# SmallVCM/SmallVCM

Hardware: AMD Instinct MI355X
Metric: Mpaths/sec (light+camera), VCM scene 1 at 2048^2 (higher is better)
Workload: dtype f32; 1 GPU; scene 1 -a vcm 2048x2048 maxPathLength 10 minPathLength 0 radiusFactor 0.003 radiusAlpha 0.75 seed 1234, iterations 5..408 timed; parallelism=1 renderer(s) (iteration-parallel, smallvcm.cxx:61-108) on one GPU, 1 in flight

## Files before the change

### smallvcm_amd/csrc/vcm_api.hip

```cpp
#include <hip/hip_runtime.h>
#include <stdio.h>
#include <stdlib.h>
#include <string.h>
#include <string>
#include <new>
#include <mutex>
#include <vector>
#include <condition_variable>
#include <atomic>

#include "vcm_kernels.h"
#include "vcm_kat.h"
#include "scene_host.h"
#include "vcm_denoise.h"
#include "vcm_variance.h"

using namespace vcm;

static thread_local std::string g_err;
static thread_local bool g_hipFailed;
static int fail(const char *what, const char *detail)
{
    g_err = std::string(what) + ": " + (detail ? detail : "");
    return -1;
// ... 188 lines not shown

static thread_local size_t g_allocBytes;
template <typename T> static int dalloc(T **p, size_t n)
{
    void *v = NULL;
    HIPCHK(hipMalloc(&v, (n ? n : 1) * sizeof(T)));
    g_allocBytes += (n ? n : 1) * sizeof(T);
    *p = (T *)v;
    return 0;
}
#define DFREE(p) do { if (p) { (void)hipFree(p); p = NULL; } } while (0)

static std::mutex g_arenaRegistryMutex;
static ArenaPool *g_pools[64];

static Arena *arena_new(int device, ArenaPool *pool)
{
    Arena *a = new Arena();
    a->device = device;
    memset((void *)&a->s, 0, sizeof(Scratch));
    a->capLocal = a->capN = 0; a->capS = a->capL = 0; a->capSharded = false; a->bytes = 0;
    a->allocated = false; a->eventReady = a->lastValid = false; a->lastUser = NULL;
    a->pool = pool; a->ownerThread = 0; a->busy = false;
    a->mtx = pool ? &pool->m : &a->ownMtx;
    a->cv = pool ? &pool->cv : &a->ownCv;
    return a;
}
static ArenaPool *pool_get(int device)
{
    if (device < 0 || device >= 64) return NULL;
    std::lock_guard<std::mutex> g(g_arenaRegistryMutex);
    if (!g_pools[device]) {
        ArenaPool *p = new ArenaPool();
        p->device = device; p->users = 0; p->count = 0;
        memset(p->arenas, 0, sizeof(p->arenas));
        const char *e = getenv("SMALLVCM_AMD_ARENAS");
        p->limit = (e && atoi(e) > 0) ? (atoi(e) < VCM_MAX_ARENAS ? atoi(e) : VCM_MAX_ARENAS) : 0;
        g_pools[device] = p;
    }
    return g_pools[device];
}

static void arena_free_buffers(Arena *a)
{
    Scratch &s = a->s;
    DFREE(s.store.v); DFREE(s.store.count); DFREE(s.store.lenMask);
    DFREE(s.dPathStart); DFREE(s.dLocalTotal); DFREE(s.dTileSums[0]); DFREE(s.dTileSums[1]); DFREE(s.dTileSums[2]); DFREE(s.dTileSums[3]);
    DFREE(s.dPixCount); DFREE(s.dPixStart); DFREE(s.dSplatArrival); DFREE(s.dSplatList);
    DFREE(s.dRecordsLocal); DFREE(s.dRecordsAll); DFREE(s.dSlotOfVertex); DFREE(s.dSplat);
    DFREE(s.dCellCount); DFREE(s.dCellStart); DFREE(s.dCellId); DFREE(s.dUnsorted); DFREE(s.dRadixHist);
    DFREE(s.dGx); DFREE(s.dGy); DFREE(s.dGz); DFREE(s.dGb); DFREE(s.dG1); DFREE(s.dG2); DFREE(s.dG3); DFREE(s.dSortedIndex);
    DFREE(s.dCamOut); DFREE(s.dCamMask);
    DFREE(s.vs.q); DFREE(s.vs.q4); DFREE(s.vs.meta); DFREE(s.vs.count);
    DFREE(s.vs.diTask); DFREE(s.vs.vcTask); DFREE(s.vs.diOut); DFREE(s.vs.vcOut); DFREE(s.vs.mergeOut);
    DFREE(s.dQueryKey); DFREE(s.dSortedVertex); DFREE(s.dQueryStart); DFREE(s.dQueryCount); DFREE(s.dQueryArrival);
    a->allocated = false;
    a->capLocal = a->capN = 0; a->capS = a->capL = 0; a->capSharded = false;
}

static int arena_ensure(Arena *a, size_t nLocal, size_t N, int S, int L, bool sharded)
{
    if (!a->eventReady) { HIPCHK(hipEventCreateWithFlags(&a->lastUse, hipEventDisableTiming)); a->eventReady = true; }
    if (a->allocated && nLocal <= a->capLocal && N <= a->capN && S <= a->capS && L <= a->capL && (!sharded || a->capSharded))
        return 0;
    HIPCHK(hipDeviceSynchronize());
    const size_t cl = nLocal > a->capLocal ? nLocal : a->capLocal, cn = N > a->capN ? N : a->capN;
    const int cs = S > a->capS ? S : a->capS, cL = L > a->capL ? L : a->capL;
    const bool sh = sharded || a->capSharded;
    arena_free_buffers(a);
    a->lastValid = false;
    a->lastUser = NULL;
    a->bytes = 0;
    const size_t bytesBefore = g_allocBytes;
    Scratch &s = a->s;
    const size_t slots = (size_t)cs * cl;
    const size_t allRecs = (size_t)cs * cn;
    if (dalloc(&s.store.v, slots * VCM_LV_FIELDS) || dalloc(&s.store.count, cl) || dalloc(&s.store.lenMask, cl)) return -1;
    if (dalloc(&s.dPathStart, cl + 1) || dalloc(&s.dLocalTotal, 1)) return -1;
    size_t maxScan = (cn > cl ? cn : cl) + 1;
    if (maxScan < (size_t)VCM_QSORT_BUCKETS + 1) maxScan = (size_t)VCM_QSORT_BUCKETS + 1;
    for (int w = 0; w < 4; w++) if (dalloc(&s.dTileSums[w], maxScan / VCM_SCAN_TILE + 2)) return -1;
    if (dalloc(&s.dRecordsLocal, slots * VCM_MERGE_RECORD_FLOATS)) return -1;
    if (dalloc(&s.dSlotOfVertex, slots) || dalloc(&s.dSplat, slots)) return -1;
    if (dalloc(&s.dPixCount, cn + 2) || dalloc(&s.dPixStart, cn + 2) || dalloc(&s.dSplatArrival, slots) || dalloc(&s.dSplatList, slots)) return -1;
    if (sh && dalloc(&s.dRecordsAll, allRecs * VCM_MERGE_RECORD_FLOATS)) return -1;
    if (dalloc(&s.dCellCount, cn + 2) || dalloc(&s.dCellStart, cn + 2)) return -1;
    if (dalloc(&s.dCellId, allRecs) || dalloc(&s.dUnsorted, allRecs) || dalloc(&s.dRadixHist, (size_t)2 * 256 * VCM_RSORT_MAX_BLOCKS)) return -1;
    if (dalloc(&s.dGx, allRecs + VCM_MERGE_UNROLL) || dalloc(&s.dGy, allRecs + VCM_MERGE_UNROLL) ||
        dalloc(&s.dGz, allRecs + VCM_MERGE_UNROLL) || dalloc(&s.dGb, 3 * (allRecs + 2 * VCM_MERGE_UNROLL)) || dalloc(&s.dG1, allRecs) || dalloc(&s.dG2, allRecs) ||
        dalloc(&s.dG3, allRecs) || dalloc(&s.dSortedIndex, allRecs)) return -1;
    if (dalloc(&s.dCamOut, cl) || dalloc(&s.dCamMask, cl) || dalloc(&s.vs.count, 32)) return -1;
    const size_t maxWaves = (size_t)VCM_MAX_TRACE_WAVES;
    const size_t vitems = (size_t)(cL > 0 ? cL : 1) * cl;
    const size_t vslots = vitems + vitems / 3 + maxWaves * VCM_QBLOCK_VERTEX;
    const size_t vcPerPath = (cL >= 3) ? (size_t)(cL - 1) * (size_t)(cL - 2) / 2 : 1;
    const size_t vcslots = 2 * vcPerPath * cl + maxWaves * VCM_QBLOCK_VC;
    s.vs.qcap = vslots;
    if (dalloc(&s.vs.q, vslots * 4) || dalloc(&s.vs.q4, vslots) || dalloc(&s.vs.meta, vslots) ||
        dalloc(&s.vs.diTask, vslots) || dalloc(&s.vs.diOut, vslots) ||
        dalloc(&s.vs.mergeOut, vslots) || dalloc(&s.vs.vcTask, 2 * vcslots) || dalloc(&s.vs.vcOut, vcslots) ||
        dalloc(&s.dQueryKey, vslots) || dalloc(&s.dSortedVertex, vslots)) return -1;
    const size_t qsN = (cn > (size_t)VCM_QSORT_BUCKETS ? cn : (size_t)VCM_QSORT_BUCKETS) + 2;
    if (dalloc(&s.dQueryStart, qsN) || dalloc(&s.dQueryCount, (size_t)VCM_QSORT_BUCKETS + 2) ||
        dalloc(&s.dQueryArrival, vslots)) return -1;
    a->capLocal = cl; a->capN = cn; a->capS = cs; a->capL = cL; a->capSharded = sh;
    a->allocated = true;
    a->bytes = g_allocBytes - bytesBefore;
    return 0;
}

static bool pool_may_grow(ArenaPool *p)
{
    if (p->count >= VCM_MAX_ARENAS) return false;
    if (p->limit > 0) return p->count < p->limit;
    if (p->count == 0) return true;
    size_t held = 0, largest = 0;
    for (int i = 0; i < p->count; i++) { held += p->arenas[i]->bytes; if (p->arenas[i]->bytes > largest) largest = p->arenas[i]->bytes; }
    size_t freeB = 0, totalB = 0;
    if (hipMemGetInfo(&freeB, &totalB) != hipSuccess) return false;
    return held + largest <= totalB / 4 && largest + (totalB / 16) <= freeB;
}

static int arena_acquire(vcm_ctx *c, int S, int L)
{
    Arena *a = NULL;
    bool wait;
    if (c->pool) {
        ArenaPool *p = c->pool;
        std::unique_lock<std::mutex> lk(p->m);
        for (;;) {
            Arena *mine = NULL, *idle = NULL, *lru = NULL;
            bool holdsOne = false;
            for (int i = 0; i < p->count; i++) {
                Arena *x = p->arenas[i];
                if (x->busy) { if (x->ownerThread == this_thread_id()) holdsOne = true; continue; }
                if (x->lastUser == c) mine = x;
                else if (!x->lastValid || hipEventQuery(x->lastUse) == hipSuccess) idle = x;
                else lru = x;
            }
            (void)hipGetLastError();
            a = mine ? mine : idle;
            if (!a && pool_may_grow(p)) { a = arena_new(p->device, p); p->arenas[p->count++] = a; }
            if (!a) a = lru;
            if (a) break;
            if (holdsOne)
                return fail("vcm_begin_iteration", "this thread is already inside an iteration on this device and no further "
                                                   "scratch arena is free: single-rank contexts share the iteration scratch, "
                                                   "end an iteration first (or raise vcm_set_arena_limit)");
            p->cv.wait(lk);
        }
        a->busy = true;
        a->ownerThread = this_thread_id();
        wait = a->lastValid && a->lastUser != c;
// ... 1098 lines not shown
        if (!c->P.wavefront && join_grid(c)) return -1;
    } else {
        if (mark(c, EV_GRID_K0)) return -1;
        if (mark(c, EV_GRID)) return -1;
    }
    return 0;
}

static GridStore grid_of(vcm_ctx *c)
{
    GridStore grid;
    grid.cellStart = c->dCellStart; grid.gx = c->dGx; grid.gy = c->dGy; grid.gz = c->dGz; grid.gb = c->dGb; grid.g1 = c->dG1; grid.g2 = c->dG2; grid.g3 = c->dG3;
    grid.hdr = c->dHdr;
    return grid;
}

static int vcm_trace_camera_impl(vcm_ctx *c)
{
    if (!c || !c->inIteration) return fail("vcm_trace_camera", "no iteration in progress");
    if (use_device(c)) return -1;
    if (flush_light_splats(c)) return -1;
    c->cameraTraced = true;
    if (c->lightTraceOnly) return 0;
    int blocks, chunk;
    trace_launch_shape(c->nLocal, &blocks, &chunk);
    if (c->resolveInFlight) HIPCHK(hipStreamWaitEvent(c->stream, c->evResolved, 0));
    if (mark(c, EV_CAMERA_K0)) return -1;
    if (c->renderer) {
        if (c->renderer == 1)
            LAUNCH_SC_CAM_PICK(c, k_path_trace, dim3(blocks), dim3(VCM_TRACE_BLOCK), 0, c->stream, c->dScene, c->P, c->dCamOut,
                               c->dRngCam, c->dStats, chunk, take_stamps(c, c->stream), c->vs.count + 8);
        else
            LAUNCH_SC_CAM(c, k_eye_light, dim3(2048), dim3(256), 0, c->stream, c->dScene, c->P, c->dCamOut, c->dRngCam,
                               c->dStats, take_stamps(c, c->stream));
        HIPCHK(hipGetLastError());
        if (mark(c, EV_CAMERA_K1)) return -1;
        if (mark(c, EV_CONNECT_K1)) return -1;
        return 0;
    }
    if (c->P.wavefront) {
        c->countedInCamera = c->useVM && (c->gridBuilt || c->bboxPreset);
        c->vs.sortHdr = c->countedInCamera ? c->dHdr : NULL;
        c->vs.sortKey = c->countedInCamera ? c->dQueryKey : NULL;
        c->vs.sortArrival = c->countedInCamera ? c->dQueryArrival : NULL;
        c->vs.bucketCount = c->countedInCamera ? c->dQueryCount : NULL;
        if (c->countedInCamera) {
            if (c->prezeroed) HIPCHK(hipStreamWaitEvent(c->stream, c->evZero, 0));
            else if (zero_ranges(c->stream, c->dQueryCount, ((size_t)c->P.nBuckets + 1) * sizeof(int))) return -1;
        }
        LAUNCH_SC_MODE_CAM_PICK(c, k_camera_trace, 1, dim3(blocks), dim3(VCM_TRACE_BLOCK), 0, c->stream, c->dScene, c->P,
                           c->store, grid_of(c), c->vs, c->dCamOut, c->dCamMask, c->dRngCam, c->dStats, chunk, take_stamps(c, c->stream));
        if (mark(c, EV_CAMERA_K1)) return -1;
        if (c->useVC) {
            c->scatteredInDI = c->countedInCamera && c->P.minLen <= 2;
            const bool inlineSort = c->scatteredInDI && (c->nLocal <= (1 << 20) || grid_sort_is_radix(c));
            if (c->countedInCamera && c->world == 1 && !inlineSort) {
                HIPCHK(hipEventRecord(c->evSortFork, c->stream));
                HIPCHK(hipStreamWaitEvent(c->side, c->evSortFork, 0));
                const StampArgs none = { { NULL, NULL, NULL, NULL } };
                if (launch_scan_on<int>(c, 3, c->side, c->dQueryCount, c->P.nBuckets, c->dQueryStart, NULL, 1, none)) return -1;
                hipLaunchKernelGGL(k_query_scatter, dim3(aux_blocks(c->nLocal)), dim3(256), 0, c->side, c->vs, (const int *)c->dQueryKey,
                                   (const int *)c->dQueryArrival, (const int *)c->dQueryStart, c->dSortedVertex);
                HIPCHK(hipEventRecord(c->evSorted, c->side));
                c->sortInFlight = true;
                c->scatteredInDI = false;
            }
            if (c->scatteredInDI && launch_scan<int>(c, c->dQueryCount, c->P.nBuckets, c->dQueryStart, NULL, 1)) return -1;
            {
                HIPCHK(hipEventRecord(c->evSplatFork, c->stream));
                HIPCHK(hipStreamWaitEvent(c->splat, c->evSplatFork, 0));
                LAUNCH_SC(c, k_connect_vc, dim3(task_blocks(c->nLocal)), dim3(VCM_TASK_BLOCK), 0, c->splat, c->dScene, c->P, c->vs,
                                   c->store, c->dStats);
                HIPCHK(hipEventRecord(c->evSplatDone, c->splat));
                c->splatInFlight = true;
            }
            LAUNCH_SC_PICK(c, k_connect_di, dim3(task_blocks(c->nLocal)), dim3(VCM_TASK_BLOCK), 0, c->stream, c->dScene, c->P, c->vs,
                               c->dStats, c->scatteredInDI ? (const int *)c->dQueryStart : (const int *)NULL,
                               c->scatteredInDI ? c->dSortedVertex : (int *)NULL, take_stamps(c, c->stream));
        }
        if (mark(c, EV_CONNECT_K1)) return -1;
    } else {
        if (c->useVM && !c->gridBuilt) return fail("vcm_trace_camera", "strict mode merges inside the camera pass: call vcm_build_grid first");
        LAUNCH_SC_MODE_CAM_PICK(c, k_camera_trace, 0, dim3(blocks), dim3(VCM_TRACE_BLOCK), 0, c->stream, c->dScene, c->P,
                           c->store, grid_of(c), c->vs, c->dCamOut, c->dCamMask, c->dRngCam, c->dStats, chunk, take_stamps(c, c->stream));
        if (mark(c, EV_CAMERA_K1)) return -1;
        if (mark(c, EV_CONNECT_K1)) return -1;
    }
    HIPCHK(hipGetLastError());
    if (c->world > 1 && flush_stamps(c, c->stream)) return -1;
    return 0;
}

#define VCM_SPACE_BLOCKS 512
static int space_scratch(vcm_ctx *c)
{
    if (c->dSpaceMatrix) return 0;
    HIPCHK(hipMalloc((void **)&c->dSpaceMatrix, sizeof(int) * VCM_SPACE_MAX_SLABS * VCM_SPACE_BLOCKS));
    HIPCHK(hipMalloc((void **)&c->dSpaceScanned, sizeof(int) * (VCM_SPACE_MAX_SLABS * VCM_SPACE_BLOCKS + 1)));
    HIPCHK(hipMalloc((void **)&c->dSpaceTotals, sizeof(int) * VCM_SPACE_MAX_SLABS));
    HIPCHK(hipMalloc((void **)&c->dSpaceHist, sizeof(int) * 256));
    return 0;
}
static int space_ready(vcm_ctx *c, const char *who)
{
    if (!c || !c->inIteration) return fail(who, "no iteration in progress");
    if (c->world <= 1) return fail(who, "the context is not sharded");
    if (!c->useVM || !c->P.wavefront) return fail(who, "needs a merging algorithm in wavefront mode");
// ... 1032 lines not shown
```

### smallvcm_amd/csrc/vcm_core.h

```cpp
#ifndef SMALLVCM_AMD_VCM_CORE_H
#define SMALLVCM_AMD_VCM_CORE_H

#include "../../include/smallvcm_amd.h"
#include "vcm_math.h"
#include "detmath.h"
#include "philox.h"

namespace vcm {

struct IterParams {
    uint32_t seed, localIter;
    uint32_t minLen, maxLen;
    int   resX, resY, N;
    int   p0, nLocal;
    int   S;
    int   useVM, useVC, lightTraceOnly, ppm;
    float radius, radiusSqr, vmNormalization, misVmWeightFactor, misVcWeightFactor;
    float lightSubPathCount;
    float cellSize, invCellSize;
    int   nCells;
    int   wavefront;
    int   renderer;
    int   iteration;
    int   qblockVertex, qblockDI, qblockVC;
    int   nBuckets;
    int   foreignOut;
};

struct GridHeader {
    uint32_t bboxMinU[3], bboxMaxU[3];
    float bboxMin[3], bboxMax[3];
    int   nRecords;
    int   nLocalRecords;
    int   pad[2];
};

#define VCM_LV_FIELDS 4
struct LightStore {
    F4 *v;
    unsigned char *count;
    uint32_t *lenMask;
};
VCM_HD F4 &lv(const LightStore &s, size_t slot, int k) { return s.v[slot * VCM_LV_FIELDS + (size_t)k]; }

struct alignas(8) F2 { float x, y; };
struct GridStore {
    const int *cellStart;
    const float *gx, *gy, *gz;
    const float *gb;
    const F4 *g1;
    const F4 *g2;
    const F2 *g3;
    const GridHeader *hdr;
};

VCM_HD size_t grid_blocked_index(int i, int axis) { return (size_t)(i >> 2) * 12u + (size_t)(axis * 4 + (i & 3)); }

struct alignas(16) I4 { int x, y, z, w; };
struct VertexStore {
    F4 *q, *q4;
    size_t qcap;
    I4 *meta;
    int *count;
    int *diTask;
    int *vcTask;
    F4 *diOut;
    F4 *vcOut;
    F4 *mergeOut;
    const GridHeader *sortHdr;
    int *sortKey, *sortArrival, *bucketCount;
};
struct alignas(8) VcTaskPair { int vertex, j; };
VCM_HD F4 &vq(const VertexStore &vs, int k, size_t i) { return k < 4 ? vs.q[i * 4 + (size_t)k] : vs.q4[i]; }
VCM_HD size_t path_slot(const IterParams &P, uint32_t pathLength, uint32_t lp)
{
    return (size_t)(pathLength - 1u) * (size_t)P.nLocal + (size_t)lp;
}
VCM_HD size_t merge_out_slot(const IterParams &P, uint32_t pathLength, uint32_t lp, int vi)
{
    return P.foreignOut ? (size_t)vi : path_slot(P, pathLength, lp);
}

struct LaneStats {
    uint32_t lightRays, cameraRays, shadowRays, mergeQueries, mergeCandidates, mergeAccepted,
             connections, lightSplats, stored;
};
VCM_HD void lane_stats_zero(LaneStats &s)
{
    s.lightRays = s.cameraRays = s.shadowRays = s.mergeQueries = s.mergeCandidates = 0;
    s.mergeAccepted = s.connections = s.lightSplats = s.stored = 0;
}

#if defined(VCM_REGION_CLOCK) && defined(__HIPCC__)
#define VCM_RC_SLOTS 2048
#define VCM_RC_IDS 64
__device__ unsigned long long g_regionClock[VCM_RC_SLOTS * 3 * VCM_RC_IDS];
#endif
#if defined(VCM_REGION_CLOCK) && defined(__HIP_DEVICE_COMPILE__)
__device__ __forceinline__ unsigned long long *rc_slot()
{
    __shared__ unsigned long long rcT[16];
    return &rcT[(threadIdx.x >> 6) & 15];
}
__device__ __forceinline__ void rc_reset() { *rc_slot() = clock64(); }
__device__ __forceinline__ void rc_mark(int id)
{
    const unsigned long long n = clock64();
    const unsigned long long m = __builtin_amdgcn_ballot_w64(true);
    unsigned long long *t = rc_slot();
    if ((int)__lane_id() == __ffsll((long long)m) - 1) {
        const unsigned long long d = n - *t;
        unsigned long long *row = g_regionClock + (size_t)((blockIdx.x * (blockDim.x >> 6) + (threadIdx.x >> 6)) & (VCM_RC_SLOTS - 1)) * (3 * VCM_RC_IDS);
        atomicAdd(&row[id], d);
        atomicAdd(&row[VCM_RC_IDS + id], 1ull);
        atomicAdd(&row[2 * VCM_RC_IDS + id], d * (unsigned long long)__popcll(m));
        *t = clock64();
    }
}
#define RC_DECL rc_reset()
#define RC_MARK(id) rc_mark(id)
#define RC_RESET rc_reset()
#else
#define RC_DECL
#define RC_MARK(id)
#define RC_RESET
#endif
// ... 2421 lines not shown
    ls.cameraRays++;
    RC_DECL;
    const bool hitSomething = scene_intersect(sc, ray, isect);
    RC_MARK(4);
    if (!hitSomething) {
        if (sc.backgroundLight >= 0) {
            if (st.pathLength >= P.minLen)
                cp.color = cp.color + st.throughput * get_light_radiance(sc, P, sc.lights()[sc.backgroundLight], sc.backgroundLight, st, ray.dir);
        }
        return false;
    }
    const V3 hitPoint = ray.org + ray.dir * isect.dist;
    isect.dist += VCM_EPS_RAY;
    Bsdf bsdf;
    bsdf_setup(bsdf, ray.dir, isect.normal, isect.matID, isect.prim, sc);
    if (bsdf.matID < 0) return false;
    {
        st.dVCM *= mis(sqr(isect.dist));
        st.dVCM /= mis(fabsf(bsdf.localDirFix.z));
        st.dVC  /= mis(fabsf(bsdf.localDirFix.z));
        st.dVM  /= mis(fabsf(bsdf.localDirFix.z));
    }
    if (isect.lightID >= 0) {
        const vcm_light &light = get_light(sc, isect.lightID);
        if (st.pathLength >= P.minLen)
            cp.color = cp.color + st.throughput * get_light_radiance(sc, P, light, isect.lightID, st, ray.dir);
        return false;
    }
    if (st.pathLength >= P.maxLen) return false;
    RC_MARK(5);

    if (MODE == 1) {
        if (!bsdf.isDelta && (P.useVC || P.useVM)) {
            uint32_t diK = 0u;
            int hasDI = 0;
            if (P.useVC && st.pathLength + 1 >= P.minLen) {
                diK = cp.rng.k;
                cp.rng.k += 3u;
                hasDI = 1;
            }
            uint32_t jmask = 0u;
            if (P.useVC) {
                const uint32_t M = cp.lightLenMask;
                const int loLen = (int)P.minLen - 1 - (int)st.pathLength;
                const int hiLen = (int)P.maxLen - 1 - (int)st.pathLength;
                if (hiLen >= 0) {
                    const uint32_t below = (loLen <= 0) ? 0u : (loLen >= 32 ? 0xffffffffu : ((1u << loLen) - 1u));
                    const uint32_t upto = (hiLen >= 31) ? 0xffffffffu : ((1u << (hiLen + 1)) - 1u);
                    const int jlo = __builtin_popcount(M & below), jhi = __builtin_popcount(M & upto);
                    if (jhi > jlo) jmask = ((jhi >= 32) ? 0xffffffffu : ((1u << jhi) - 1u)) & ~((1u << jlo) - 1u);
                }
            }
            const int nvc = __builtin_popcount(jmask);
#if defined(__HIP_DEVICE_COMPILE__)
            const unsigned long long act = __builtin_amdgcn_ballot_w64(true);
            const int rank = (int)lanes_below_mask_popc(act);
            int vb = wq_load(wqs.v.p), vl = wq_load(wqs.v.p + 1), db = wq_load(wqs.di.p), dl = wq_load(wqs.di.p + 1), cb = wq_load(wqs.vc.p), cl = wq_load(wqs.vc.p + 1);
            const int vi = wave_queue_take<0>(vb, vl, &vs.count[0], P.qblockVertex, 1, act, rank,
                [&](int first, int cnt, int rk, int na) {
                    for (int i = rk; i < cnt; i += na) {
                        vq(vs, 0, first + i) = mk4(0.f, 0.f, 0.f, u2f(0xffffffffu));
                        if (vs.sortKey) vs.sortKey[first + i] = -1;
                    } });
            const int di = wave_queue_take<1>(db, dl, &vs.count[1], P.qblockDI, hasDI, act, rank,
                [&](int first, int cnt, int rk, int na) { for (int i = rk; i < cnt; i += na) vs.diTask[first + i] = -1; });
            const int vc0 = wave_queue_take<5>(cb, cl, &vs.count[2], P.qblockVC, nvc, act, rank,
                [&](int first, int cnt, int rk, int na) { for (int i = rk; i < cnt; i += na) vs.vcTask[2 * (first + i)] = -1; });
            if (rank == 0) { wq_store(wqs.v.p, vb); wq_store(wqs.v.p + 1, vl); wq_store(wqs.di.p, db); wq_store(wqs.di.p + 1, dl); wq_store(wqs.vc.p, cb); wq_store(wqs.vc.p + 1, cl); }
#else
            const int vi = wave_queue_alloc(wqs.v, &vs.count[0], P.qblockVertex, 1, [](int, int, int, int) {});
            const int di = wave_queue_alloc(wqs.di, &vs.count[1], P.qblockDI, hasDI, [](int, int, int, int) {});
            const int vc0 = wave_queue_alloc(wqs.vc, &vs.count[2], P.qblockVC, nvc, [](int, int, int, int) {});
#endif
            vq(vs, 0, vi) = mk4(hitPoint.x, hitPoint.y, hitPoint.z, u2f((uint32_t)cp.lp));
            vq(vs, 1, vi) = mk4(isect.normal.x, isect.normal.y, isect.normal.z, u2f(st.pathLength | (shade_code(bsdf.matID, isect.prim) << 8)));
            vq(vs, 2, vi) = mk4(bsdf.localDirFix.x, bsdf.localDirFix.y, bsdf.localDirFix.z, st.dVCM);
            vq(vs, 3, vi) = mk4(st.throughput.x, st.throughput.y, st.throughput.z, st.dVM);
            vq(vs, 4, vi) = mk4(st.dVC, u2f(diK), 0.f, 0.f);
            I4 m; m.x = hasDI ? di : -1; m.y = vc0; m.z = nvc; m.w = 0;
            vs.meta[path_slot(P, st.pathLength, (uint32_t)cp.lp)] = m;
#if defined(__HIP_DEVICE_COMPILE__)
            if (vs.sortKey && P.useVM) {
                const int k = query_sort_key(P, qk, hitPoint);
                vs.sortKey[vi] = k;
#if defined(VCM_NO_DEFER)
                if (k >= 0) vs.sortArrival[vi] = atomicAdd(&vs.bucketCount[k], 1);
#else
                if (wqs.pendingVertex >= 0) vs.sortArrival[wqs.pendingVertex] = wqs.pendingArrival;
                wqs.pendingVertex = -1;
                if (k >= 0) { wqs.pendingVertex = vi; wqs.pendingArrival = atomicAdd(&vs.bucketCount[k], 1); }
#endif
                else vs.mergeOut[path_slot(P, st.pathLength, (uint32_t)cp.lp)] = mk4(0.f, 0.f, 0.f, 0.f);
            }
#endif
            if (hasDI) vs.diTask[di] = vi;
            int t = vc0;
            while (jmask) {
                const int j = __builtin_ctz(jmask);
                jmask &= jmask - 1u;
                VcTaskPair pr; pr.vertex = vi; pr.j = j;
                reinterpret_cast<VcTaskPair *>(vs.vcTask)[t] = pr;
                t++;
            }
            cp.queryMask |= 1u << st.pathLength;
            if (P.useVM) {
                ls.mergeQueries++;
                if (P.ppm) return false;
            }
        }
    } else {
        if (!bsdf.isDelta && P.useVC) {
            if (st.pathLength + 1 >= P.minLen) {
                float rnd[3];
                rng_peek(cp.rng, cp.rng.k, rnd, 3);
                cp.rng.k += 3u;
                cp.color = cp.color + st.throughput * direct_illumination(sc, P, rnd[0], rnd[1], rnd[2], st, hitPoint, bsdf, ls);
            }
        }
        if (!bsdf.isDelta && P.useVC) {
            const int n = store.count[cp.lp];
            for (int j = 0; j < n; j++) {
                const size_t slot = (size_t)j * (size_t)P.nLocal + (size_t)cp.lp;
                const F4 a = lv(store, slot, 0);
                const uint32_t lvLen = f2u(a.w) & 0xffu;
                if (lvLen + 1 + st.pathLength < P.minLen) continue;
                if (lvLen + 1 + st.pathLength > P.maxLen) break;
                const F4 b = lv(store, slot, 1);
                const F4 c = lv(store, slot, 2);
                const F4 d = lv(store, slot, 3);
                Bsdf lvBsdf;
                bsdf_restore(lvBsdf, mk3(c.x, c.y, c.z), mk3(d.x, d.y, d.z), f2u(a.w) >> 8, sc);
                cp.color = cp.color + st.throughput * mk3(b.x, b.y, b.z) *
                           connect_vertices(sc, P, mk3(a.x, a.y, a.z), lvBsdf, b.w, c.w, bsdf, hitPoint, st, ls);
            }
        }
        if (!bsdf.isDelta && P.useVM) {
            ls.mergeQueries++;
            const V3 contrib = merge_query<SC::kIntPhong>(sc, P, grid, bsdf, st, hitPoint, ls, ms);
            cp.color = cp.color + st.throughput * P.vmNormalization * contrib;
            if (P.ppm) return false;
        }
    }
    RC_MARK(6);
    const bool goesOn = sample_scattering(sc, P, false, cp.rng, bsdf, hitPoint, st);
    RC_MARK(7);
    if (!goesOn) return false;
    ++st.pathLength;
    return true;
}

struct CamVertex {
    V3 hit, throughput;
    Bsdf bsdf;
    SubPathState st;
    uint32_t lp;
    uint32_t diK;
// ... 260 lines not shown
```

### smallvcm_amd/csrc/vcm_kernels.h

```cpp
#ifndef SMALLVCM_AMD_VCM_KERNELS_H
#define SMALLVCM_AMD_VCM_KERNELS_H

#include <hip/hip_runtime.h>
#include "vcm_core.h"

namespace vcm {

enum { STAT_LIGHT_RAYS = 0, STAT_CAMERA_RAYS, STAT_SHADOW_RAYS, STAT_MERGE_QUERIES, STAT_MERGE_CANDIDATES,
       STAT_MERGE_ACCEPTED, STAT_CONNECTIONS, STAT_LIGHT_SPLATS, STAT_STORED, STAT_COUNT };

#define VCM_TRACE_BLOCK 256
#define VCM_WAVE 64

struct StampArgs { unsigned long long *p[4]; };
__device__ __forceinline__ void stamp_entry(const StampArgs &s)
{
    if (blockIdx.x == 0 && threadIdx.x == 0 && s.p[0]) {
        const unsigned long long t = wall_clock64();
#pragma unroll
        for (int k = 0; k < 4; k++) if (s.p[k]) *s.p[k] = t;
    }
}

__device__ __forceinline__ unsigned lane_id() { return __builtin_amdgcn_mbcnt_hi(~0u, __builtin_amdgcn_mbcnt_lo(~0u, 0u)); }
// ... 118 lines not shown
#if defined(VCM_K3_WAVES)
#define VCM_K3_ATTR __attribute__((amdgpu_waves_per_eu(VCM_K3_WAVES, VCM_K3_WAVES)))
#else
#define VCM_K3_ATTR
#endif
template <int MODE, class SC>
__global__ void __launch_bounds__(VCM_TRACE_BLOCK) VCM_K3_ATTR
k_camera_trace(const DScene *__restrict__ scp, IterParams P, LightStore store, GridStore grid, VertexStore vs,
               F4 *camOut, uint32_t *camMask, unsigned char *rngCount, unsigned long long *gstats, int chunk, StampArgs st)
{
    stamp_entry(st);
    const SC &sc = *static_cast<const SC *>(scp);
    stage_scene_tables(sc);
    stage_pick_tables(sc);
    const unsigned lane = lane_id();
    WaveWork ww; wave_work_init(ww, chunk, P.nLocal);
    int *work = vs.count + 8;
    LaneStats ls; lane_stats_zero(ls);
    __shared__ uint32_t accQ[MODE == 1 ? 1 : (VCM_MERGE_Q + 1) * VCM_TRACE_BLOCK];
    MergeScratch ms; ms.q = accQ + (MODE == 1 ? 0 : threadIdx.x); ms.stride = VCM_TRACE_BLOCK; ms.cap = VCM_MERGE_Q;
    __shared__ int wqState[(VCM_TRACE_BLOCK / VCM_WAVE) * 6];
    int *myState = wqState + (threadIdx.x / VCM_WAVE) * 6;
    if (lane < 6) myState[lane] = 0;
    CameraWaveQueues wqs;
    wqs.v.p = (WaveQueueWords)myState; wqs.di.p = (WaveQueueWords)(myState + 2); wqs.vc.p = (WaveQueueWords)(myState + 4);
    wqs.pendingVertex = -1; wqs.pendingArrival = 0;
    QueryKey qk = { 0.f, 0.f, 0.f, 0.f, 0.f, 0.f, 1u, 1u, 0, 0, 0 };
    if (MODE == 1 && vs.sortKey && P.useVM) qk = query_key_load(P, vs.sortHdr);
    CameraPath path;
    bool alive = false;
    RC_DECL;
    for (;;) {
        const unsigned long long need = __builtin_amdgcn_ballot_w64(!alive);
        if (need) {
            const int idx = wave_work_take(ww, work, chunk, P.nLocal, need, lane);
            if (!alive && idx >= 0) { camera_path_begin(sc, P, path, idx, MODE == 1 ? store.lenMask : (const uint32_t *)0); alive = true; }
        }
        RC_MARK(20);
        if (!wave_any(alive)) { if (ww.exhausted) break; else continue; }
        if (alive) {
            alive = camera_path_step<MODE>(sc, P, path, store, grid, ls, ms, vs, wqs, qk);
            RC_RESET;
            if (!alive) {
                const int target = camera_path_target(P, path);
                camOut[path.lp] = mk4(path.color.x, path.color.y, path.color.z, u2f((uint32_t)target));
                if (MODE == 1) camMask[path.lp] = path.queryMask;
                rngCount[path.lp] = (unsigned char)path.rng.k;
            }
        }
        RC_MARK(22);
    }
    if (MODE == 1 && wqs.pendingVertex >= 0) vs.sortArrival[wqs.pendingVertex] = wqs.pendingArrival;
    if (MODE == 1) {
        const int vb = wq_load(wqs.v.p), vl = wq_load(wqs.v.p + 1), db = wq_load(wqs.di.p), dl = wq_load(wqs.di.p + 1), cb = wq_load(wqs.vc.p), cl = wq_load(wqs.vc.p + 1);
        for (int i = (int)lane; i < vl; i += VCM_WAVE) {
            vq(vs, 0, vb + i) = mk4(0.f, 0.f, 0.f, u2f(0xffffffffu));
            if (vs.sortKey) vs.sortKey[vb + i] = -1;
        }
        for (int i = (int)lane; i < dl; i += VCM_WAVE) vs.diTask[db + i] = -1;
        for (int i = (int)lane; i < cl; i += VCM_WAVE) vs.vcTask[2 * (cb + i)] = -1;
    }
    flush_stats(ls, gstats);
}

template <class SC>
__global__ void __launch_bounds__(VCM_TRACE_BLOCK)
k_path_trace(const DScene *__restrict__ scp, IterParams P, F4 *camOut, unsigned char *rngCount,
             unsigned long long *gstats, int chunk, StampArgs st, int *work)
{
    stamp_entry(st);
    const SC &sc = *static_cast<const SC *>(scp);
    stage_scene_tables(sc);
    stage_pick_tables(sc);
    const unsigned lane = lane_id();
    WaveWork ww; wave_work_init(ww, chunk, P.nLocal);
    LaneStats ls; lane_stats_zero(ls);
    PtPath path;
    bool alive = false;
    for (;;) {
        const unsigned long long need = __builtin_amdgcn_ballot_w64(!alive);
        if (need) {
            const int idx = wave_work_take(ww, work, chunk, P.nLocal, need, lane);
            if (!alive && idx >= 0) { pt_path_begin(sc, P, path, idx); alive = true; }
        }
        if (!wave_any(alive)) { if (ww.exhausted) break; else continue; }
        if (alive) {
            alive = pt_path_step(sc, P, path, ls);
            if (!alive) {
                camOut[path.lp] = mk4(path.color.x, path.color.y, path.color.z, u2f((uint32_t)raster_target(P, path.sx, path.sy)));
                rngCount[path.lp] = (unsigned char)path.rng.k;
            }
        }
    }
    flush_stats(ls, gstats);
}

template <class SC>
__global__ void __launch_bounds__(256)
k_eye_light(const DScene *__restrict__ scp, IterParams P, F4 *camOut, unsigned char *rngCount,
            unsigned long long *gstats, StampArgs st)
{
    stamp_entry(st);
    const SC &sc = *static_cast<const SC *>(scp);
    stage_scene_tables(sc);
    LaneStats ls; lane_stats_zero(ls);
    for (int lp = blockIdx.x * blockDim.x + threadIdx.x; lp < P.nLocal; lp += gridDim.x * blockDim.x) {
        V3 color = sp3(0.f);
        float sx, sy;
        uint32_t drawn;
        const bool hit = eyelight_path(sc, P, lp, color, sx, sy, drawn, ls);
        camOut[lp] = mk4(color.x, color.y, color.z, u2f((uint32_t)(hit ? raster_target(P, sx, sy) : -1)));
        rngCount[lp] = (unsigned char)drawn;
    }
    flush_stats(ls, gstats);
}

#define VCM_TASK_BLOCK 256
#if defined(VCM_TASK_WAVES)
#define VCM_TASK_ATTR __attribute__((amdgpu_waves_per_eu(VCM_TASK_WAVES, VCM_TASK_WAVES)))
#else
#define VCM_TASK_ATTR
#endif
template <class SC>
__global__ void __launch_bounds__(VCM_TASK_BLOCK) VCM_TASK_ATTR
k_connect_di(const DScene *__restrict__ scp, IterParams P, VertexStore vs, unsigned long long *gstats,
             const int *__restrict__ bucketStart, int *sortedVertex, StampArgs st)
{
    stamp_entry(st);
    const SC &sc = *static_cast<const SC *>(scp);
    stage_scene_tables(sc);
    stage_pick_tables(sc);
    const int n = vs.count[1];
    LaneStats ls; lane_stats_zero(ls);
    for (int t = blockIdx.x * VCM_TASK_BLOCK + threadIdx.x; t < n; t += gridDim.x * VCM_TASK_BLOCK) {
        const int vi = vs.diTask[t];
        if (vi < 0) continue;
        size_t ps;
        const V3 v = eval_di_task(sc, P, vs, vi, ls, ps);
        vs.diOut[ps] = mk4(v.x, v.y, v.z, 0.f);
        if (sortedVertex) {
            const int k = vs.sortKey[vi];
            if (k >= 0) sortedVertex[bucketStart[k] + vs.sortArrival[vi]] = vi;
        }
    }
    flush_stats(ls, gstats);
}

template <class SC>
__global__ void __launch_bounds__(VCM_TASK_BLOCK) VCM_TASK_ATTR
k_connect_vc(const DScene *__restrict__ scp, IterParams P, VertexStore vs, LightStore store,
             unsigned long long *gstats)
{
    const SC &sc = *static_cast<const SC *>(scp);
    stage_scene_tables(sc);
    const int n = vs.count[2];
    LaneStats ls; lane_stats_zero(ls);
    for (int t = blockIdx.x * VCM_TASK_BLOCK + threadIdx.x; t < n; t += gridDim.x * VCM_TASK_BLOCK) {
        const VcTaskPair pr = reinterpret_cast<const VcTaskPair *>(vs.vcTask)[t];
        const int vi = pr.vertex;
        if (vi < 0) continue;
        const V3 v = eval_vc_task(sc, P, vs, store, vi, pr.j, ls);
        vs.vcOut[t] = mk4(v.x, v.y, v.z, 0.f);
    }
    flush_stats(ls, gstats);
}


__global__ void __launch_bounds__(256) k_query_count(IterParams P, VertexStore vs, const GridHeader *__restrict__ hdr, int *key, int *arrival,
                              int *bucketCount, StampArgs st)
{
    stamp_entry(st);
    const int nQ = vs.count[0];
    for (int q = blockIdx.x * blockDim.x + threadIdx.x; q < nQ; q += gridDim.x * blockDim.x) {
        const F4 r0 = vq(vs, 0, q);
        int k = -1;
        if (f2u(r0.w) != 0xffffffffu) {
            k = query_sort_key(P, hdr, mk3(r0.x, r0.y, r0.z));
            if (k < 0)
                vs.mergeOut[merge_out_slot(P, f2u(vq(vs, 1, q).w) & 0xffu, f2u(r0.w), q)] = mk4(0.f, 0.f, 0.f, 0.f);
        }
        key[q] = k;
        if (k >= 0) arrival[q] = atomicAdd(&bucketCount[k], 1);
    }
}

__global__ void __launch_bounds__(256) k_query_scatter(VertexStore vs, const int *__restrict__ key, const int *__restrict__ arrival,
                                const int *__restrict__ bucketStart, int *sortedVertex)
{
    const int nQ = vs.count[0];
    for (int q = blockIdx.x * blockDim.x + threadIdx.x; q < nQ; q += gridDim.x * blockDim.x) {
        const int k = key[q];
        if (k >= 0) sortedVertex[bucketStart[k] + arrival[q]] = q;
    }
}

#ifndef VCM_MERGE_BLOCK
#define VCM_MERGE_BLOCK 256
#endif

#if defined(VCM_K4_WAVES)
#define VCM_K4_ATTR __attribute__((amdgpu_waves_per_eu(VCM_K4_WAVES, VCM_K4_WAVES)))
#else
#define VCM_K4_ATTR
#endif
#ifndef VCM_WALK_Q
#define VCM_WALK_Q 20
#endif
#if defined(__HIP_DEVICE_COMPILE__)
struct alignas(8) WalkRun { int lo, hi; };
__device__ __forceinline__ int merge_walk_runs(const IterParams &P, const GridStore &g, V3 queryPos, WalkRun *runs ,
                                               int stride, int &total)
{
    int n = 0;
    total = 0;
    const V3 bmin = ld3(g.hdr->bboxMin), bmax = ld3(g.hdr->bboxMax);
// ... 1328 lines not shown
```

Baseline: 1229 Mpaths/s.

## Derive DI and VC connection tasks from vertex queue instead of separate task queues

Drops the separate diTask and vcTask queues and their atomic slot allocation and hole-filling in the camera trace. Each vertex record now packs its VC output base, task count, first light index and a has-DI flag into its fifth slot. The DI kernel scans the vertex queue and checks the flag. The VC kernel expands per-vertex task counts into per-lane tasks with a wave-level ballot prefix sum and a shared-memory carry buffer. This saves queue allocation and writes in the trace kernel, but adds per-wave scan work and assumes the light-vertex indices for a vertex's VC tasks are contiguous starting at the lowest set bit.

```diff
diff --git a/smallvcm_amd/csrc/vcm_api.hip b/smallvcm_amd/csrc/vcm_api.hip
--- a/smallvcm_amd/csrc/vcm_api.hip
+++ b/smallvcm_amd/csrc/vcm_api.hip
@@ -264,7 +264,7 @@
     DFREE(s.dGx); DFREE(s.dGy); DFREE(s.dGz); DFREE(s.dGb); DFREE(s.dG1); DFREE(s.dG2); DFREE(s.dG3); DFREE(s.dSortedIndex);
     DFREE(s.dCamOut); DFREE(s.dCamMask);
     DFREE(s.vs.q); DFREE(s.vs.q4); DFREE(s.vs.meta); DFREE(s.vs.count);
-    DFREE(s.vs.diTask); DFREE(s.vs.vcTask); DFREE(s.vs.diOut); DFREE(s.vs.vcOut); DFREE(s.vs.mergeOut);
+    DFREE(s.vs.diOut); DFREE(s.vs.vcOut); DFREE(s.vs.mergeOut);
     DFREE(s.dQueryKey); DFREE(s.dSortedVertex); DFREE(s.dQueryStart); DFREE(s.dQueryCount); DFREE(s.dQueryArrival);
     a->allocated = false;
     a->capLocal = a->capN = 0; a->capS = a->capL = 0; a->capSharded = false;
@@ -309,8 +309,8 @@
     const size_t vcslots = 2 * vcPerPath * cl + maxWaves * VCM_QBLOCK_VC;
     s.vs.qcap = vslots;
     if (dalloc(&s.vs.q, vslots * 4) || dalloc(&s.vs.q4, vslots) || dalloc(&s.vs.meta, vslots) ||
-        dalloc(&s.vs.diTask, vslots) || dalloc(&s.vs.diOut, vslots) ||
-        dalloc(&s.vs.mergeOut, vslots) || dalloc(&s.vs.vcTask, 2 * vcslots) || dalloc(&s.vs.vcOut, vcslots) ||
+        dalloc(&s.vs.diOut, vslots) ||
+        dalloc(&s.vs.mergeOut, vslots) || dalloc(&s.vs.vcOut, vcslots) ||
         dalloc(&s.dQueryKey, vslots) || dalloc(&s.dSortedVertex, vslots)) return -1;
     const size_t qsN = (cn > (size_t)VCM_QSORT_BUCKETS ? cn : (size_t)VCM_QSORT_BUCKETS) + 2;
     if (dalloc(&s.dQueryStart, qsN) || dalloc(&s.dQueryCount, (size_t)VCM_QSORT_BUCKETS + 2) ||
@@ -1515,7 +1515,7 @@
                            c->store, grid_of(c), c->vs, c->dCamOut, c->dCamMask, c->dRngCam, c->dStats, chunk, take_stamps(c, c->stream));
         if (mark(c, EV_CAMERA_K1)) return -1;
         if (c->useVC) {
-            c->scatteredInDI = c->countedInCamera && c->P.minLen <= 2;
+            c->scatteredInDI = c->countedInCamera;
             const bool inlineSort = c->scatteredInDI && (c->nLocal <= (1 << 20) || grid_sort_is_radix(c));
             if (c->countedInCamera && c->world == 1 && !inlineSort) {
                 HIPCHK(hipEventRecord(c->evSortFork, c->stream));
diff --git a/smallvcm_amd/csrc/vcm_core.h b/smallvcm_amd/csrc/vcm_core.h
--- a/smallvcm_amd/csrc/vcm_core.h
+++ b/smallvcm_amd/csrc/vcm_core.h
@@ -62,16 +62,21 @@
     size_t qcap;
     I4 *meta;
     int *count;
-    int *diTask;
-    int *vcTask;
     F4 *diOut;
     F4 *vcOut;
     F4 *mergeOut;
     const GridHeader *sortHdr;
     int *sortKey, *sortArrival, *bucketCount;
 };
-struct alignas(8) VcTaskPair { int vertex, j; };
 VCM_HD F4 &vq(const VertexStore &vs, int k, size_t i) { return k < 4 ? vs.q[i * 4 + (size_t)k] : vs.q4[i]; }
+VCM_HD uint32_t vertex_task_word(int nvc, int jlo, int hasDI) { return (uint32_t)nvc | ((uint32_t)jlo << 8) | ((uint32_t)hasDI << 16); }
+#define VCM_VERTEX_HAS_DI 0x10000u
+VCM_HD void vertex_queue_mark_hole(const VertexStore &vs, size_t i)
+{
+    vq(vs, 0, i) = mk4(0.f, 0.f, 0.f, u2f(0xffffffffu));
+    vs.q4[i] = mk4(0.f, 0.f, 0.f, 0.f);
+    if (vs.sortKey) vs.sortKey[i] = -1;
+}
 VCM_HD size_t path_slot(const IterParams &P, uint32_t pathLength, uint32_t lp)
 {
     return (size_t)(pathLength - 1u) * (size_t)P.nLocal + (size_t)lp;
@@ -2599,33 +2604,29 @@
                 }
             }
             const int nvc = __builtin_popcount(jmask);
+            const int jlo = nvc ? __builtin_ctz(jmask) : 0;
+            RC_MARK(47);
 #if defined(__HIP_DEVICE_COMPILE__)
             const unsigned long long act = __builtin_amdgcn_ballot_w64(true);
             const int rank = (int)lanes_below_mask_popc(act);
-            int vb = wq_load(wqs.v.p), vl = wq_load(wqs.v.p + 1), db = wq_load(wqs.di.p), dl = wq_load(wqs.di.p + 1), cb = wq_load(wqs.vc.p), cl = wq_load(wqs.vc.p + 1);
+            int vb = wq_load(wqs.v.p), vl = wq_load(wqs.v.p + 1), cb = wq_load(wqs.vc.p), cl = wq_load(wqs.vc.p + 1);
             const int vi = wave_queue_take<0>(vb, vl, &vs.count[0], P.qblockVertex, 1, act, rank,
-                [&](int first, int cnt, int rk, int na) {
-                    for (int i = rk; i < cnt; i += na) {
-                        vq(vs, 0, first + i) = mk4(0.f, 0.f, 0.f, u2f(0xffffffffu));
-                        if (vs.sortKey) vs.sortKey[first + i] = -1;
-                    } });
-            const int di = wave_queue_take<1>(db, dl, &vs.count[1], P.qblockDI, hasDI, act, rank,
-                [&](int first, int cnt, int rk, int na) { for (int i = rk; i < cnt; i += na) vs.diTask[first + i] = -1; });
-            const int vc0 = wave_queue_take<5>(cb, cl, &vs.count[2], P.qblockVC, nvc, act, rank,
-                [&](int first, int cnt, int rk, int na) { for (int i = rk; i < cnt; i += na) vs.vcTask[2 * (first + i)] = -1; });
-            if (rank == 0) { wq_store(wqs.v.p, vb); wq_store(wqs.v.p + 1, vl); wq_store(wqs.di.p, db); wq_store(wqs.di.p + 1, dl); wq_store(wqs.vc.p, cb); wq_store(wqs.vc.p + 1, cl); }
+                [&](int first, int cnt, int rk, int na) { for (int i = rk; i < cnt; i += na) vertex_queue_mark_hole(vs, first + i); });
+            const int vc0 = wave_queue_take<5>(cb, cl, &vs.count[2], P.qblockVC, nvc, act, rank, [](int, int, int, int) {});
+            if (rank == 0) { wq_store(wqs.v.p, vb); wq_store(wqs.v.p + 1, vl); wq_store(wqs.vc.p, cb); wq_store(wqs.vc.p + 1, cl); }
 #else
             const int vi = wave_queue_alloc(wqs.v, &vs.count[0], P.qblockVertex, 1, [](int, int, int, int) {});
-            const int di = wave_queue_alloc(wqs.di, &vs.count[1], P.qblockDI, hasDI, [](int, int, int, int) {});
             const int vc0 = wave_queue_alloc(wqs.vc, &vs.count[2], P.qblockVC, nvc, [](int, int, int, int) {});
 #endif
+            RC_MARK(42);
             vq(vs, 0, vi) = mk4(hitPoint.x, hitPoint.y, hitPoint.z, u2f((uint32_t)cp.lp));
             vq(vs, 1, vi) = mk4(isect.normal.x, isect.normal.y, isect.normal.z, u2f(st.pathLength | (shade_code(bsdf.matID, isect.prim) << 8)));
             vq(vs, 2, vi) = mk4(bsdf.localDirFix.x, bsdf.localDirFix.y, bsdf.localDirFix.z, st.dVCM);
             vq(vs, 3, vi) = mk4(st.throughput.x, st.throughput.y, st.throughput.z, st.dVM);
-            vq(vs, 4, vi) = mk4(st.dVC, u2f(diK), 0.f, 0.f);
-            I4 m; m.x = hasDI ? di : -1; m.y = vc0; m.z = nvc; m.w = 0;
+            vq(vs, 4, vi) = mk4(st.dVC, u2f(diK), u2f((uint32_t)vc0), u2f(vertex_task_word(nvc, jlo, hasDI)));
+            I4 m; m.x = hasDI ? 0 : -1; m.y = vc0; m.z = nvc; m.w = 0;
             vs.meta[path_slot(P, st.pathLength, (uint32_t)cp.lp)] = m;
+            RC_MARK(43);
 #if defined(__HIP_DEVICE_COMPILE__)
             if (vs.sortKey && P.useVM) {
                 const int k = query_sort_key(P, qk, hitPoint);
@@ -2640,15 +2641,7 @@
                 else vs.mergeOut[path_slot(P, st.pathLength, (uint32_t)cp.lp)] = mk4(0.f, 0.f, 0.f, 0.f);
             }
 #endif
-            if (hasDI) vs.diTask[di] = vi;
-            int t = vc0;
-            while (jmask) {
-                const int j = __builtin_ctz(jmask);
-                jmask &= jmask - 1u;
-                VcTaskPair pr; pr.vertex = vi; pr.j = j;
-                reinterpret_cast<VcTaskPair *>(vs.vcTask)[t] = pr;
-                t++;
-            }
+            RC_MARK(44);
             cp.queryMask |= 1u << st.pathLength;
             if (P.useVM) {
                 ls.mergeQueries++;
diff --git a/smallvcm_amd/csrc/vcm_kernels.h b/smallvcm_amd/csrc/vcm_kernels.h
--- a/smallvcm_amd/csrc/vcm_kernels.h
+++ b/smallvcm_amd/csrc/vcm_kernels.h
@@ -194,13 +194,8 @@
     }
     if (MODE == 1 && wqs.pendingVertex >= 0) vs.sortArrival[wqs.pendingVertex] = wqs.pendingArrival;
     if (MODE == 1) {
-        const int vb = wq_load(wqs.v.p), vl = wq_load(wqs.v.p + 1), db = wq_load(wqs.di.p), dl = wq_load(wqs.di.p + 1), cb = wq_load(wqs.vc.p), cl = wq_load(wqs.vc.p + 1);
-        for (int i = (int)lane; i < vl; i += VCM_WAVE) {
-            vq(vs, 0, vb + i) = mk4(0.f, 0.f, 0.f, u2f(0xffffffffu));
-            if (vs.sortKey) vs.sortKey[vb + i] = -1;
-        }
-        for (int i = (int)lane; i < dl; i += VCM_WAVE) vs.diTask[db + i] = -1;
-        for (int i = (int)lane; i < cl; i += VCM_WAVE) vs.vcTask[2 * (cb + i)] = -1;
+        const int vb = wq_load(wqs.v.p), vl = wq_load(wqs.v.p + 1);
+        for (int i = (int)lane; i < vl; i += VCM_WAVE) vertex_queue_mark_hole(vs, (size_t)(vb + i));
     }
     flush_stats(ls, gstats);
 }
@@ -272,14 +267,15 @@
     const SC &sc = *static_cast<const SC *>(scp);
     stage_scene_tables(sc);
     stage_pick_tables(sc);
-    const int n = vs.count[1];
+    const int n = vs.count[0];
     LaneStats ls; lane_stats_zero(ls);
-    for (int t = blockIdx.x * VCM_TASK_BLOCK + threadIdx.x; t < n; t += gridDim.x * VCM_TASK_BLOCK) {
-        const int vi = vs.diTask[t];
-        if (vi < 0) continue;
-        size_t ps;
-        const V3 v = eval_di_task(sc, P, vs, vi, ls, ps);
-        vs.diOut[ps] = mk4(v.x, v.y, v.z, 0.f);
+    for (int vi = blockIdx.x * VCM_TASK_BLOCK + threadIdx.x; vi < n; vi += gridDim.x * VCM_TASK_BLOCK) {
+        if (f2u(vq(vs, 0, vi).w) == 0xffffffffu) continue;
+        if (f2u(vs.q4[vi].w) & VCM_VERTEX_HAS_DI) {
+            size_t ps;
+            const V3 v = eval_di_task(sc, P, vs, vi, ls, ps);
+            vs.diOut[ps] = mk4(v.x, v.y, v.z, 0.f);
+        }
         if (sortedVertex) {
             const int k = vs.sortKey[vi];
             if (k >= 0) sortedVertex[bucketStart[k] + vs.sortArrival[vi]] = vi;
@@ -295,14 +291,62 @@
 {
     const SC &sc = *static_cast<const SC *>(scp);
     stage_scene_tables(sc);
-    const int n = vs.count[2];
+    constexpr int W = VCM_TASK_BLOCK / VCM_WAVE;
+    __shared__ int sSum[W][VCM_WAVE];
+    __shared__ int sCarryV[W][VCM_WAVE], sCarryK[W][VCM_WAVE];
+    const int lane = (int)lane_id(), wave = (int)threadIdx.x / VCM_WAVE;
+    int *sum = sSum[wave], *carryV = sCarryV[wave], *carryK = sCarryK[wave];
+    const int n = wave_uniform(vs.count[0]);
+    const int nGroups = (n + VCM_WAVE - 1) / VCM_WAVE, nWaves = (int)gridDim.x * W;
     LaneStats ls; lane_stats_zero(ls);
-    for (int t = blockIdx.x * VCM_TASK_BLOCK + threadIdx.x; t < n; t += gridDim.x * VCM_TASK_BLOCK) {
-        const VcTaskPair pr = reinterpret_cast<const VcTaskPair *>(vs.vcTask)[t];
-        const int vi = pr.vertex;
-        if (vi < 0) continue;
-        const V3 v = eval_vc_task(sc, P, vs, store, vi, pr.j, ls);
-        vs.vcOut[t] = mk4(v.x, v.y, v.z, 0.f);
+    int carryN = 0;
+    for (int g = (int)blockIdx.x * W + wave;; g += nWaves) {
+        const bool last = g >= nGroups;
+        const int vi0 = g * VCM_WAVE;
+        int cnt = 0;
+        if (!last && vi0 + lane < n) cnt = (int)(f2u(vs.q4[vi0 + lane].w) & 0xffu);
+        int before = 0, total = 0;
+#pragma unroll
+        for (int bit = 0; bit < 5; bit++) {
+            const unsigned long long m = __builtin_amdgcn_ballot_w64(((cnt >> bit) & 1) != 0);
+            before += (int)lanes_below_mask_popc(m) << bit;
+            total += __popcll(m) << bit;
+        }
+        __builtin_amdgcn_wave_barrier();
+        sum[lane] = before + cnt;
+        __builtin_amdgcn_wave_barrier();
+        const int have = carryN + total;
+        const int run = last ? have : (have & ~(VCM_WAVE - 1));
+        for (int c0 = 0; c0 < run; c0 += VCM_WAVE) {
+            const int c = c0 + lane;
+            if (c < run) {
+                int tv, tk;
+                if (c < carryN) { tv = carryV[c]; tk = carryK[c]; }
+                else {
+                    const int id = c - carryN;
+                    int src = 0;
+#pragma unroll
+                    for (int s = VCM_WAVE / 2; s; s >>= 1) if (sum[src + s - 1] <= id) src += s;
+                    tv = vi0 + src;
+                    tk = id - (src ? sum[src - 1] : 0);
+                }
+                const F4 e = vs.q4[tv];
+                const V3 v = eval_vc_task(sc, P, vs, store, tv, (int)((f2u(e.w) >> 8) & 0xffu) + tk, ls);
+                vs.vcOut[(size_t)((int)f2u(e.z) + tk)] = mk4(v.x, v.y, v.z, 0.f);
+            }
+        }
+        if (last) break;
+        const int c = (run > carryN ? run : carryN) + lane;
+        __builtin_amdgcn_wave_barrier();
+        if (c < have) {
+            const int id = c - carryN;
+            int src = 0;
+#pragma unroll
+            for (int s = VCM_WAVE / 2; s; s >>= 1) if (sum[src + s - 1] <= id) src += s;
+            carryV[c - run] = vi0 + src;
+            carryK[c - run] = id - (src ? sum[src - 1] : 0);
+        }
+        carryN = have - run;
     }
     flush_stats(ls, gstats);
 }
```

Result: faster. 1242 Mpaths/s (median of 6 runs) (+1.1%).
